# google/neural-light-transport

Hardware: AMD Instinct MI355X
Metric: rendered Mtexels/s at 1024^2 UV (full Model.call forward: U-Net + UV->camera warp); at N > 1: N collective-free replicas of this forward (weak scaling).  The data-parallel TRAIN step with the RCCL gradient all-reduce (BASELINE config 4) is `train_step`: value = Mtexels/s over all ranks, speedup_vs_o (higher is better)
Workload: dtype f32 via 3xbf16 split, 9 exact products, fp32 accumulate (the LDS-tiled encoder convs: fp32 operands as three bf16 terms on v_mfma_f32_16x16x32_bf16, every term product exact in fp32); f32 storage everywhere, every other launch native f32; 1 GPU; BASELINE config 3: dragon_specular relight+view-synth, depth0 16/depth 256, 4 frames/GPU, 1024^2 UV, k=4 obs maps, 512^2 camera warp; frames_per_gpu=4, uv=1024, k=4, cam=512, conv_algo=auto, plan=fused ends, launch=eager, two HIP streams, distinct_batches_rotated=3, launch_tape_replays=0, parallelism=dp1 (frames sharded, no forward collective), world=1, dist_world_size=1, device=cuda:0

## Files before the change

neural-light-transport_amd/csrc/conv_tile3.hip:

```cpp
#include "nlt_common.h"
#include "pack_common.h"

namespace {

typedef __attribute__((ext_vector_type(8))) __bf16 bf16x8;
typedef unsigned short u16;
typedef unsigned int u32x4 __attribute__((ext_vector_type(4)));

constexpr int TH = 8, TW = 16;
constexpr int QS2 = 272, ODD2 = 132;
constexpr int PL = 160;

template <int MODE> struct T3;
template <> struct T3<NLT_CONV_K2S1> { static constexpr int PAIRS = 2, B_UNITS = 153 * 2, B_SLOTS = 6 * PL; };
template <> struct T3<NLT_CONV_K2S2> { static constexpr int PAIRS = 1, B_UNITS = 256 * 2, B_SLOTS = 6 * QS2; };

struct Tile3P {
  const float* src; const u16* packed; const float* bias;
  float* out; float* mean_out;
  int ld, cin, frames, kobs, h, w;
  int oh, ow, cout, ldo, ldm;
  int tiles_y, tiles_x, ncc;
  int act; float alpha;
};

__device__ __forceinline__ int xcd_tile3(int b, int nblocks) {
  return (nblocks & 7) ? b : (b & 7) * (nblocks >> 3) + (b >> 3);
}

__device__ __forceinline__ unsigned cvt_pk_bf16(float a, float b) {
  typedef float f32x2_ __attribute__((ext_vector_type(2)));
  typedef __bf16 bf16x2_ __attribute__((ext_vector_type(2)));
  return __builtin_bit_cast(unsigned, __builtin_convertvector((f32x2_){a, b}, bf16x2_));
}

__device__ __forceinline__ void split2(float a, float b, unsigned& hi, unsigned& mid, unsigned& lo) {
  hi = cvt_pk_bf16(a, b);
  const float ra = a - __uint_as_float(hi << 16), rb = b - __uint_as_float(hi & 0xffff0000u);
  mid = cvt_pk_bf16(ra, rb);
  const float sa = ra - __uint_as_float(mid << 16), sb = rb - __uint_as_float(mid & 0xffff0000u);
  lo = cvt_pk_bf16(sa, sb);
}

__device__ __forceinline__ void split8(const f32x4& v0, const f32x4& v1, u32x4& hi, u32x4& mid, u32x4& lo) {
  unsigned h[4], m[4], l[4];
  split2(v0[0], v0[1], h[0], m[0], l[0]);
  split2(v0[2], v0[3], h[1], m[1], l[1]);
  split2(v1[0], v1[1], h[2], m[2], l[2]);
  split2(v1[2], v1[3], h[3], m[3], l[3]);
  hi = (u32x4){h[0], h[1], h[2], h[3]};
  mid = (u32x4){m[0], m[1], m[2], m[3]};
  lo = (u32x4){l[0], l[1], l[2], l[3]};
}


__device__ __forceinline__ int unit_half(int u) { return (u >> 3) & 1; }
__device__ __forceinline__ int unit_texel(int u) { return (u >> 4) * 8 + (u & 7); }

__device__ __forceinline__ void gather_unit(const float* sp, int ld, bool ok, long tex, int hf, f32x4& v0, f32x4& v1) {
  const float* q8 = sp + (ok ? tex : 0) * ld + 8 * hf;
  const f32x4 g0 = *reinterpret_cast<const f32x4*>(q8), g1 = *reinterpret_cast<const f32x4*>(q8 + 4);
  const f32x4 z = {0.f, 0.f, 0.f, 0.f};
  v0 = ok ? g0 : z;
  v1 = ok ? g1 : z;
}

__device__ __forceinline__ void split_store_unit(u32x4* bb, int bpl, const f32x4& v0, const f32x4& v1) {
  u32x4 hi, mid, lo;
  split8(v0, v1, hi, mid, lo);
  bb[0] = hi;
  bb[2 * bpl] = mid;
  bb[4 * bpl] = lo;
}

__device__ __forceinline__ void wave_sync() {
  __builtin_amdgcn_fence(__ATOMIC_RELEASE, "wavefront");
  __builtin_amdgcn_wave_barrier();
  __builtin_amdgcn_fence(__ATOMIC_ACQUIRE, "wavefront");
}

template <int CT>
__device__ __forceinline__ void read_a(const u32x4* A, int tile0, int lane, bf16x8 (&at)[3][CT]) {
#pragma unroll
  for (int ct = 0; ct < CT; ++ct)
#pragma unroll
    for (int t = 0; t < 3; ++t) at[t][ct] = __builtin_bit_cast(bf16x8, A[((tile0 + ct) * 3 + t) * 64 + lane]);
}

constexpr int ORDER9[9][2] = {{2, 2}, {2, 1}, {1, 2}, {2, 0}, {0, 2}, {1, 1}, {1, 0}, {0, 1}, {0, 0}};

template <int NPROD, int NR, int CT, class BFrag>
__device__ __forceinline__ void term_products(const bf16x8 (&at)[3][CT], BFrag bfrag, f32x4 (&acc)[NR][CT]) {
#pragma unroll
  for (int pi = 9 - NPROD; pi < 9; ++pi)
#pragma unroll
    for (int r = 0; r < NR; ++r)
#pragma unroll
      for (int ct = 0; ct < CT; ++ct)
        acc[r][ct] = __builtin_amdgcn_mfma_f32_16x16x32_bf16(at[ORDER9[pi][0]][ct], bfrag(ORDER9[pi][1], r), acc[r][ct], 0, 0, 0);
}

__device__ __forceinline__ f32x4 bias_act(const f32x4& acc, const f32x4& bv, int act, float alpha) {
  f32x4 v = acc + bv;
  if (act) {
#pragma unroll
    for (int c4 = 0; c4 < 4; ++c4) v[c4] = v[c4] > 0.f ? v[c4] : alpha * v[c4];
  }
  return v;
}

__host__ __device__ inline u16 bf16_rne_bits(float f) {
  union { float f; unsigned u; } x; x.f = f;
  x.u += 0x7fffu + ((x.u >> 16) & 1u);
  return (u16)(x.u >> 16);
}
__host__ __device__ inline float bf16_bits_float(u16 b) {
  union { float f; unsigned u; } x; x.u = (unsigned)b << 16;
  return x.f;
}

__global__ void pack_tile3_kernel(const float* __restrict__ wk, int cin, int cout, int tnt, long total, u16* __restrict__ wp) {
  const long idx = (long)blockIdx.x * blockDim.x + threadIdx.x;
  if (idx >= total) return;
  const int e = idx & 7, lane = (idx >> 3) & 63;
  long r = idx >> 9;
  const int term = r % 3; r /= 3;
  const int ct = r % tnt; r /= tnt;
  const int pair = r & 1; r >>= 1;
  const int ncc = cin >> 4;
  const int cc = r % ncc;
  const int g = r / ncc;
  const int kk = lane >> 4, i = lane & 15;
  const int t = pair * 2 + (kk >> 1);
  const int c = cc * 16 + (kk & 1) * 8 + e;
  const int o = (g * tnt + ct) * 16 + i;
  const float v = wk[((long)t * cin + c) * cout + o];
  const u16 hi = bf16_rne_bits(v);
  const float r1 = v - bf16_bits_float(hi);
  const u16 mid = bf16_rne_bits(r1);
  const float r2 = r1 - bf16_bits_float(mid);
  wp[idx] = term == 0 ? hi : (term == 1 ? mid : bf16_rne_bits(r2));
}

template <bool NEXT_ITEM, int NR, int CT>
__device__ __forceinline__ void epilogue(const Tile3P& p, int f, int i, int oc0, int gy0, int gx, f32x4 (&acc)[NR][CT],
                                         f32x4 (&mean)[NR][CT]) {
#pragma unroll
  for (int ct = 0; ct < CT; ++ct) {
    const int oc = oc0 + 16 * ct;
    const f32x4 bv = *reinterpret_cast<const f32x4*>(p.bias + oc);
#pragma unroll
    for (int r = 0; r < NR; ++r) {
      const int gy = gy0 + r;
      const f32x4 v = bias_act(acc[r][ct], bv, p.act, p.alpha);
      acc[r][ct] = (f32x4){0.f, 0.f, 0.f, 0.f};
      mean[r][ct] += v;
      if (gy < p.oh && gx < p.ow) {
        const long ot = ((long)(f * p.kobs + i) * p.oh + gy) * p.ow + gx;
        if (p.out) *reinterpret_cast<f32x4*>(p.out + ot * p.ldo + oc) = v;
        if (p.mean_out && i == p.kobs - 1) {
          const long mt = ((long)f * p.oh + gy) * p.ow + gx;
          *reinterpret_cast<f32x4*>(p.mean_out + mt * p.ldm + oc) = mean[r][ct] * (1.f / (float)p.kobs);
        }
      }
      if (NEXT_ITEM && i == p.kobs - 1) mean[r][ct] = (f32x4){0.f, 0.f, 0.f, 0.f};
    }
  }
}

template <int MODE>
__device__ __forceinline__ void unit_slot(int u, int& hf, int& slot, bool& st) {
  const int tx = unit_texel(u);
  hf = unit_half(u);
  if (MODE == NLT_CONV_K2S1) {
    st = tx < 153;
    slot = hf * PL + tx;
  } else {
    const int y = tx >> 5, xx = tx & 31;
    st = tx < 256;
    slot = hf * QS2 + (xx & 1) * ODD2 + y * 16 + (xx >> 1);
  }
}
template <int MODE>
__device__ __forceinline__ void unit_source(const Tile3P& p, int tx, bool st, int ty0, int tx0, bool& ok, long& tex) {
  if (MODE == NLT_CONV_K2S1) {
    const int gy = ty0 + tx / 17, gx = tx0 + tx % 17;
    ok = st && gy < p.h && gx < p.w;
    tex = (long)gy * p.w + gx;
  } else {
    const int y = tx >> 5, xx = tx & 31;
    const int gy = 2 * (ty0 + y), gx = 2 * tx0 + xx;
    ok = st && (ty0 + y) < p.oh && gx < p.w;
    tex = (long)gy * p.w + gx;
  }
}
template <int MODE, int TNT, int NPROD, int RT, int CT>
__device__ __forceinline__ void stage_products(const u32x4* A, const u32x4* B, int lane, int wm, int wn, f32x4 (&acc)[RT][CT]) {
  constexpr int BPL = MODE == NLT_CONV_K2S1 ? PL : QS2;
  const int kk = lane >> 4, j = lane & 15;
#pragma unroll
  for (int pl = 0; pl < T3<MODE>::PAIRS; ++pl) {
    bf16x8 bt[3][RT], at[3][CT];
#pragma unroll
    for (int rt = 0; rt < RT; ++rt) {
      const int y = wm * RT + rt;
      const int slot = MODE == NLT_CONV_K2S1 ? (kk & 1) * PL + (y + pl) * 17 + j + (kk >> 1)
                                             : (kk & 1) * QS2 + (kk >> 1) * ODD2 + y * 16 + j;
#pragma unroll
      for (int t = 0; t < 3; ++t) bt[t][rt] = __builtin_bit_cast(bf16x8, B[t * 2 * BPL + slot]);
    }
    read_a(A, pl * TNT + wn * CT, lane, at);
    term_products<NPROD>(at, [&](int t, int rt) { return bt[t][rt]; }, acc);
  }
}

template <int MODE, int TNT, int NPROD, int KO>
__global__ __launch_bounds__(256, 2) void conv_tile3_kernel(Tile3P p) {
  using TT = T3<MODE>;
  constexpr int WN = TNT == 4 ? 2 : 1, WM = 4 / WN, RT = TH / WM, CT = 2;
  constexpr int A_SLOTS = TT::PAIRS * TNT * 3 * 64;
  constexpr int NA = (A_SLOTS + 255) / 256, NB = (TT::B_UNITS + 255) / 256;
// ... 190 lines not shown
#pragma unroll
            for (int e = 0; e < KO; ++e)
              epilogue<true>(p, f, gi * KO + e, (g * TNT + wn * CT) * 16 + 4 * kk, ty0 + wm * RT, tx0 + j, acc[e], mean);
          }
          if (!(item_end && last_item)) store_b((q + 1) & 1);
          __syncthreads();
        }
      }
    }
    if (!last_item && ng != g) {
      copy_a(ng);
      __syncthreads();
    }
  }
}

constexpr size_t TILE3R_LDS_CU = 160 * 1024;

int tile3r_cus() {
  static const int n = [] {
    int dev = 0, v = 0;
    if (hipGetDevice(&dev) != hipSuccess) return 0;
    if (hipDeviceGetAttribute(&v, hipDeviceAttributeMultiprocessorCount, dev) != hipSuccess) return 0;
    return v;
  }();
  return n;
}

long tile3r_grid(int per_cu, int max_wg, long items) {
  long nwg = (long)tile3r_cus() * per_cu;
  if (max_wg > 0 && nwg > max_wg) nwg = max_wg;
  return nwg > items ? items : nwg;
}

int tile3r_allow_lds(const void* kernel, size_t lds, size_t (&done)[8]) {
  int dev = 0;
  if (lds <= 64 * 1024) return NLT_OK;
  if (hipGetDevice(&dev) != hipSuccess) return NLT_ERR_LAUNCH;
  if (dev >= 0 && dev < 8 && done[dev] >= lds) return NLT_OK;
  if (hipFuncSetAttribute(kernel, hipFuncAttributeMaxDynamicSharedMemorySize, (int)lds) != hipSuccess) return NLT_ERR_LAUNCH;
  if (dev >= 0 && dev < 8) done[dev] = lds;
  return NLT_OK;
}

template <int MODE, int TNT, int NPROD, int KO, int NWV>
int launch3r_k(const Tile3P& p, size_t lds, int nwg, hipStream_t s) {
  auto* k = conv_tile3r_kernel<MODE, TNT, NPROD, KO, NWV>;
  static size_t done[8] = {};
  if (tile3r_allow_lds(reinterpret_cast<const void*>(k), lds, done) != NLT_OK) return NLT_ERR_LAUNCH;
  hipLaunchKernelGGL(k, dim3((unsigned)nwg), dim3(64 * NWV), lds, s, p, p.cout / (16 * TNT));
  NLT_CHECK_LAUNCH();
  return NLT_OK;
}

template <int RT, int NPROD>
__global__ __launch_bounds__(512, 2) void conv_tile3w_kernel(Tile3P p, int ngroups, int tiles_y) {
  constexpr int TNT = 2, CT = 2, NWV = 8;
  constexpr int ROWS = RT + 1, UNITS = ROWS * 17 * 2, NB = (UNITS + 63) / 64;
  constexpr int PLW = (ROWS * 17 + 15) / 16 * 16;
  constexpr int A_SLOTS = 2 * TNT * 3 * 64;
  const int a_group = p.ncc * A_SLOTS;
  const int tid = threadIdx.x, lane = tid & 63, wave = tid >> 6;
  const int kk = lane >> 4, j = lane & 15;
  u32x4* const B = tile3r_lds + a_group + wave * (6 * PLW);
  const long in_frame = (long)p.h * p.w;
  const int tiles = p.frames * tiles_y * p.tiles_x;
  const long items = (long)tiles * ngroups;
  const int rank = xcd_tile3(blockIdx.x, gridDim.x);
  const int it0 = (int)(rank * items / gridDim.x), it1 = (int)((rank + 1) * items / gridDim.x);

  int b_lds[NB], b_hf[NB], b_tx[NB]; long b_tex[NB]; bool b_ok[NB], b_st[NB];
#pragma unroll
  for (int i = 0; i < NB; ++i) {
    b_hf[i] = unit_half(lane + 64 * i);
    b_tx[i] = unit_texel(lane + 64 * i);
    b_st[i] = b_tx[i] < ROWS * 17;
    b_lds[i] = b_hf[i] * PLW + b_tx[i];
  }
  int nf = 0, nty0 = 0, ntx0 = 0;
  auto geom = [&](int t) {
    ntx0 = (t % p.tiles_x) * TW; t /= p.tiles_x;
    nty0 = (t % tiles_y) * RT;
    nf = t / tiles_y;
#pragma unroll
    for (int i = 0; i < NB; ++i) unit_source<NLT_CONV_K2S1>(p, b_tx[i], b_st[i], nty0, ntx0, b_ok[i], b_tex[i]);
  };
  f32x4 rb[NB][2];
  auto load_b = [&](int cc, int frame) {
    const float* sp = p.src + (long)(nf * p.kobs + frame) * in_frame * p.ld + cc * 16;
#pragma unroll
    for (int n = 0; n < NB; ++n) gather_unit(sp, p.ld, b_ok[n], b_tex[n], b_hf[n], rb[n][0], rb[n][1]);
  };
  auto store_b = [&]() {
#pragma unroll
    for (int n = 0; n < NB; ++n)
      if (b_st[n]) split_store_unit(B + b_lds[n], PLW, rb[n][0], rb[n][1]);
  };

  int seg = it0;
  while (seg < it1) {
    const int g = seg / tiles;
    const int seg_end = min(it1, (g + 1) * tiles);
    {
      const u32x4* ap = reinterpret_cast<const u32x4*>(p.packed) + (long)g * a_group;
      for (int i = tid; i < a_group; i += 64 * NWV) tile3r_lds[i] = ap[i];
    }
    __syncthreads();
    int it = seg + wave;
    if (it < seg_end) {
      f32x4 acc[RT][CT], mean[RT][CT];
#pragma unroll
      for (int rt = 0; rt < RT; ++rt)
#pragma unroll
        for (int ct = 0; ct < CT; ++ct) acc[rt][ct] = mean[rt][ct] = (f32x4){0.f, 0.f, 0.f, 0.f};
      geom(it - g * tiles);
      load_b(0, 0);
      store_b();
      wave_sync();
      for (; it < seg_end; it += NWV) {
        const int f = nf, ty0 = nty0, tx0 = ntx0;
        const bool last_item = it + NWV >= seg_end;
        for (int i = 0; i < p.kobs; ++i) {
          for (int s = 0; s < p.ncc; ++s) {
            int ns = s + 1, ni = i;
            if (ns == p.ncc) { ns = 0; ++ni; }
            const bool item_end = ni == p.kobs;
            if (item_end) {
              ni = 0;
              if (!last_item) geom(it + NWV - g * tiles);
            }
            load_b(ns, ni);
            bf16x8 bt[3][ROWS];
#pragma unroll
            for (int r = 0; r < ROWS; ++r)
#pragma unroll
              for (int t = 0; t < 3; ++t)
                bt[t][r] = __builtin_bit_cast(bf16x8, B[t * 2 * PLW + (kk & 1) * PLW + r * 17 + j + (kk >> 1)]);
            wave_sync();
            const u32x4* A = tile3r_lds + s * A_SLOTS;
#pragma unroll
            for (int pl = 0; pl < 2; ++pl) {
              bf16x8 at[3][CT];
              read_a(A, pl * TNT, lane, at);
              term_products<NPROD>(at, [&](int t, int rt) { return bt[t][rt + pl]; }, acc);
            }
            if (!(item_end && last_item)) store_b();
            wave_sync();
            if (s == p.ncc - 1) epilogue<true>(p, f, i, g * TNT * 16 + 4 * kk, ty0, tx0 + j, acc, mean);
          }
        }
      }
    }
    seg = seg_end;
    if (seg < it1) __syncthreads();
  }
}

template <int RT>
int launch3w(const Tile3P& p, int nprod, int max_wg, hipStream_t s) {
  constexpr int PLW = ((RT + 1) * 17 + 15) / 16 * 16;
  const size_t lds = (size_t)p.cin * 2 * 384 + 8 * 6 * PLW * sizeof(u32x4);
  if (lds > TILE3R_LDS_CU) return NLT_ERR_UNSUPPORTED;
  const int tiles_y = (p.oh + RT - 1) / RT;
  const long nwg = tile3r_grid(1, max_wg, (long)p.frames * tiles_y * p.tiles_x * (p.cout / 32));
  if (nwg <= 0) return NLT_ERR_LAUNCH;
  auto* k = nprod == 9 ? conv_tile3w_kernel<RT, 9> : conv_tile3w_kernel<RT, 6>;
  static size_t done[2][8] = {};
  if (tile3r_allow_lds(reinterpret_cast<const void*>(k), lds, done[nprod == 9]) != NLT_OK) return NLT_ERR_LAUNCH;
  hipLaunchKernelGGL(k, dim3((unsigned)nwg), dim3(512), lds, s, p, p.cout / 32, tiles_y);
  NLT_CHECK_LAUNCH();
  return NLT_OK;
}

template <int MODE, int TNT, int KO>
int launch3r(const Tile3P& p, int nprod, int max_wg, hipStream_t s) {
  if (nprod != 6 && nprod != 9) return NLT_ERR_UNSUPPORTED;
  if (MODE == NLT_CONV_K2S1 && TNT == 2) {
    int st = launch3w<4>(p, nprod, max_wg, s);
    if (st == NLT_ERR_UNSUPPORTED) st = launch3w<2>(p, nprod, max_wg, s);
    if (st != NLT_ERR_UNSUPPORTED) return st;
  }
  const size_t lds = (size_t)p.cin * TNT * 384 + 2 * T3<MODE>::B_SLOTS * sizeof(u32x4);
  if (lds > TILE3R_LDS_CU) return NLT_ERR_UNSUPPORTED;
  const bool wide = 2 * lds > TILE3R_LDS_CU;
  const long items = (long)p.frames * p.tiles_y * p.tiles_x * (p.cout / (16 * TNT));
  const int nwg = (int)tile3r_grid(wide ? 1 : 2, max_wg, items);
  if (nwg <= 0) return NLT_ERR_LAUNCH;
  if (items >= (1l << 31)) return NLT_ERR_UNSUPPORTED;
  if (wide) return nprod == 9 ? launch3r_k<MODE, TNT, 9, KO, 8>(p, lds, nwg, s) : launch3r_k<MODE, TNT, 6, KO, 8>(p, lds, nwg, s);
  return nprod == 9 ? launch3r_k<MODE, TNT, 9, KO, 4>(p, lds, nwg, s) : launch3r_k<MODE, TNT, 6, KO, 4>(p, lds, nwg, s);
}

template <int MODE, int TNT, int KO>
int launch3k(const Tile3P& p, int nprod, hipStream_t s, int resident_wg) {
  if (resident_wg >= 0) return launch3r<MODE, TNT, KO>(p, nprod, resident_wg, s);
  const long tiles = (long)p.frames * p.tiles_y * p.tiles_x;
  const dim3 grid((unsigned)tiles, (unsigned)(p.cout / (16 * TNT)));
  if (nprod == 9) hipLaunchKernelGGL((conv_tile3_kernel<MODE, TNT, 9, KO>), grid, dim3(256), 0, s, p);
  else if (nprod == 6) hipLaunchKernelGGL((conv_tile3_kernel<MODE, TNT, 6, KO>), grid, dim3(256), 0, s, p);
  else if (KO > 1) return NLT_ERR_UNSUPPORTED;
  else if (nprod == 3) hipLaunchKernelGGL((conv_tile3_kernel<MODE, TNT, 3, 1>), grid, dim3(256), 0, s, p);
  else hipLaunchKernelGGL((conv_tile3_kernel<MODE, TNT, 1, 1>), grid, dim3(256), 0, s, p);
  NLT_CHECK_LAUNCH();
  return NLT_OK;
}

template <int MODE, int TNT>
int launch3(const Tile3P& p, int nprod, hipStream_t s, int resident_wg) {
  static const int want = [] { const char* e = getenv("NLT_TILE3_KO"); return e ? atoi(e) : 0; }();
  const int cap = want > 0 ? want : (TNT == 2 ? 4 : (MODE == NLT_CONV_K2S1 || resident_wg >= 0 ? 1 : 2));
  if (nprod >= 6) {
    if (TNT == 2 && cap >= 4 && p.kobs % 4 == 0) return launch3k<MODE, TNT, (TNT == 2 ? 4 : 1)>(p, nprod, s, resident_wg);
    if (cap >= 2 && p.kobs % 2 == 0) return launch3k<MODE, TNT, 2>(p, nprod, s, resident_wg);
  }
  return launch3k<MODE, TNT, 1>(p, nprod, s, resident_wg);
}

constexpr int S2_PITCH = 20, S2_ODD = 9, S2_PLW = 112;
constexpr int S2_A1 = 2 * 2 * 2 * 3 * 64, S2_A2 = 4 * 4 * 3 * 64;
constexpr size_t S2_LDS = (size_t)(S2_A1 + S2_A2 + 8 * 6 * S2_PLW) * sizeof(u32x4) + 96 * sizeof(float);

struct Tile3S2P {
  Tile3P a;
  const u16* packed2; const float* bias2; float* out2;
  int ldo2, act2; float alpha2;
};

template <int NPROD>
__global__ __launch_bounds__(512, 2) void conv_tile3w_s2_kernel(Tile3S2P P, int tiles_y) {
  const Tile3P& p = P.a;
  constexpr int RT = 4, CT = 2, NWV = 8, NCL = 4, NC2 = 4;
  constexpr int UNITS = 5 * 17 * 2, NB = (UNITS + 63) / 64;
  constexpr int A_SLOTS = S2_A1 / 2;
  const int tid = threadIdx.x, lane = tid & 63, wave = tid >> 6;
  const int kk = lane >> 4, j = lane & 15, yq = j >> 3, xq = j & 7;
  const u32x4* const A2 = tile3r_lds + S2_A1;
  u32x4* const B = tile3r_lds + S2_A1 + S2_A2 + wave * (6 * S2_PLW);
  float* const biasl = reinterpret_cast<float*>(tile3r_lds + S2_A1 + S2_A2 + 8 * 6 * S2_PLW);
  const long in_frame = (long)p.h * p.w;
  const int oh2 = p.h >> 1, ow2 = p.w >> 1;
  const long items = (long)p.frames * tiles_y * p.tiles_x;
  const int rank = xcd_tile3(blockIdx.x, gridDim.x);
  const int it0 = (int)(rank * items / gridDim.x), it1 = (int)((rank + 1) * items / gridDim.x);

  int b_lds[NB], b_hf[NB], b_row[NB], b_x[NB]; long b_tex[NB]; bool b_ok[NB], b_st[NB];
#pragma unroll
  for (int i = 0; i < NB; ++i) {
    const int t = unit_texel(lane + 64 * i), q = t % 17;
    b_hf[i] = unit_half(lane + 64 * i);
    b_row[i] = t / 17;
    b_x[i] = q < S2_ODD ? 2 * q : 2 * (q - S2_ODD) + 1;
    b_st[i] = t < 5 * 17;
    b_lds[i] = b_hf[i] * S2_PLW + b_row[i] * S2_PITCH + q;
  }
  int nf = 0, nty0 = 0, ntx0 = 0;
  auto geom = [&](int t) {
    ntx0 = (t % p.tiles_x) * TW; t /= p.tiles_x;
    nty0 = (t % tiles_y) * RT;
    nf = t / tiles_y;
#pragma unroll
    for (int i = 0; i < NB; ++i) {
      const int gy = nty0 + b_row[i], gx = ntx0 + b_x[i];
      b_ok[i] = b_st[i] && gy < p.h && gx < p.w;
      b_tex[i] = (long)gy * p.w + gx;
    }
  };
  f32x4 rb[NB][2];
  auto load_b = [&](int cc, int frame) {
    const float* sp = p.src + (long)(nf * p.kobs + frame) * in_frame * p.ld + cc * 16;
#pragma unroll
    for (int n = 0; n < NB; ++n) gather_unit(sp, p.ld, b_ok[n], b_tex[n], b_hf[n], rb[n][0], rb[n][1]);
  };
  auto store_b = [&]() {
#pragma unroll
    for (int n = 0; n < NB; ++n)
      if (b_st[n]) split_store_unit(B + b_lds[n], S2_PLW, rb[n][0], rb[n][1]);
  };

  {
    const u32x4* a1 = reinterpret_cast<const u32x4*>(p.packed);
    const u32x4* a2 = reinterpret_cast<const u32x4*>(P.packed2);
    for (int i = tid; i < S2_A1; i += 64 * NWV) tile3r_lds[i] = a1[i];
    for (int i = tid; i < S2_A2; i += 64 * NWV) tile3r_lds[S2_A1 + i] = a2[i];
    if (tid < 32) biasl[tid] = p.bias[tid];
    else if (tid < 96) biasl[tid] = P.bias2[tid - 32];
  }
  __syncthreads();
  int it = it0 + wave;
  if (it >= it1) return;
  const int bl0 = (kk & 1) * S2_PLW + 2 * yq * S2_PITCH + xq;
  int offx[2];
#pragma unroll
  for (int tx = 0; tx < 2; ++tx) {
    const int xx = tx + (kk >> 1);
    offx[tx] = (xx & 1) * S2_ODD + (xx >> 1);
  }
  f32x4 acc[NCL][CT], mean[NCL][CT];
#pragma unroll
  for (int c = 0; c < NCL; ++c)
#pragma unroll
    for (int ct = 0; ct < CT; ++ct) acc[c][ct] = mean[c][ct] = (f32x4){0.f, 0.f, 0.f, 0.f};
  geom(it);
  load_b(0, 0);
  store_b();
  wave_sync();
  for (; it < it1; it += NWV) {
    const int f = nf, ty0 = nty0, tx0 = ntx0;
    const bool last_item = it + NWV >= it1;
    for (int i = 0; i < p.kobs; ++i) {
      for (int s = 0; s < 2; ++s) {
        int ns = s + 1, ni = i;
        if (ns == 2) { ns = 0; ++ni; }
        const bool item_end = ni == p.kobs;
        if (item_end) {
          ni = 0;
          if (!last_item) geom(it + NWV);
        }
        load_b(ns, ni);
        bf16x8 bt[3][6];
#pragma unroll
        for (int rs = 0; rs < 3; ++rs)
#pragma unroll
          for (int tx = 0; tx < 2; ++tx)
#pragma unroll
            for (int t = 0; t < 3; ++t)
              bt[t][rs * 2 + tx] = __builtin_bit_cast(bf16x8, B[t * 2 * S2_PLW + bl0 + rs * S2_PITCH + offx[tx]]);
        wave_sync();
        const u32x4* A = tile3r_lds + s * A_SLOTS;
#pragma unroll
        for (int pl = 0; pl < 2; ++pl) {
          bf16x8 at[3][CT];
          read_a(A, pl * 2, lane, at);
          term_products<NPROD>(at, [&](int t, int c) { return bt[t][((c >> 1) + pl) * 2 + (c & 1)]; }, acc);
        }
        if (s == 1) {
          u32x4 bs[3][NCL];
#pragma unroll
          for (int c = 0; c < NCL; ++c) {
            const int gy = ty0 + 2 * yq + (c >> 1), gx = tx0 + 2 * xq + (c & 1);
            f32x4 v2[CT];
#pragma unroll
            for (int ct = 0; ct < CT; ++ct) {
              const int oc = ct * 16 + 4 * kk;
              const f32x4 v = bias_act(acc[c][ct], *reinterpret_cast<const f32x4*>(biasl + oc), p.act, p.alpha);
              acc[c][ct] = (f32x4){0.f, 0.f, 0.f, 0.f};
              mean[c][ct] += v;
              if (p.mean_out && i == p.kobs - 1 && gy < p.oh && gx < p.ow) {
                const long mt = ((long)f * p.oh + gy) * p.ow + gx;
                *reinterpret_cast<f32x4*>(p.mean_out + mt * p.ldm + oc) = mean[c][ct] * (1.f / (float)p.kobs);
              }
              if (i == p.kobs - 1) mean[c][ct] = (f32x4){0.f, 0.f, 0.f, 0.f};
              v2[ct] = v;
            }
            split8(v2[0], v2[1], bs[0][c], bs[1][c], bs[2][c]);
          }
          f32x4 acc2[NC2 / 2][1][2];
#pragma unroll
          for (int c2 = 0; c2 < NC2; ++c2) acc2[c2 >> 1][0][c2 & 1] = (f32x4){0.f, 0.f, 0.f, 0.f};
#pragma unroll
          for (int c = 0; c < NCL; ++c) {
#pragma unroll
            for (int ch = 0; ch < NC2; ch += 2) {
              bf16x8 a2[3][2];
              read_a(A2, c * NC2 + ch, lane, a2);
              term_products<NPROD>(a2, [&](int t, int) { return __builtin_bit_cast(bf16x8, bs[t][c]); }, acc2[ch >> 1]);
            }
          }
          const int oy = (ty0 >> 1) + yq, ox = (tx0 >> 1) + xq;
          if (oy < oh2 && ox < ow2) {
            const long ot = ((long)(f * p.kobs + i) * oh2 + oy) * ow2 + ox;
#pragma unroll
            for (int c2 = 0; c2 < NC2; ++c2) {
              const int oc = c2 * 16 + 4 * kk;
              *reinterpret_cast<f32x4*>(P.out2 + ot * P.ldo2 + oc) =
                  bias_act(acc2[c2 >> 1][0][c2 & 1], *reinterpret_cast<const f32x4*>(biasl + 32 + oc), P.act2, P.alpha2);
            }
          }
        }
        if (!(item_end && last_item)) store_b();
        wave_sync();
      }
    }
  }
}

int launch3w_s2(const Tile3S2P& P, int nprod, int max_wg, hipStream_t s) {
  if (S2_LDS > TILE3R_LDS_CU) return NLT_ERR_UNSUPPORTED;
  const int tiles_y = (P.a.oh + 3) / 4;
  const long items = (long)P.a.frames * tiles_y * P.a.tiles_x;
  const long nwg = tile3r_grid(1, max_wg, items);
  if (nwg <= 0) return NLT_ERR_LAUNCH;
  if (items >= (1l << 31)) return NLT_ERR_UNSUPPORTED;
  auto* k = nprod == 9 ? conv_tile3w_s2_kernel<9> : conv_tile3w_s2_kernel<6>;
  static size_t done[2][8] = {};
  if (tile3r_allow_lds(reinterpret_cast<const void*>(k), S2_LDS, done[nprod == 9]) != NLT_OK) return NLT_ERR_LAUNCH;
  hipLaunchKernelGGL(k, dim3((unsigned)nwg), dim3(512), S2_LDS, s, P, tiles_y);
  NLT_CHECK_LAUNCH();
  return NLT_OK;
}

__global__ void pack_tile3s2_kernel(const float* __restrict__ wk, int cin, int cout, long total, u16* __restrict__ wp) {
  const long idx = (long)blockIdx.x * blockDim.x + threadIdx.x;
  if (idx < total) wp[idx] = nlt_tile3s2_fragment(wk, idx, cin, cout);
}

int tile3_params(Tile3P& p, bool own_args, bool supported, bool own_layout, int ld_other, bool stride2,
                 const float* src, int ld, int cin, int frames, int kobs, int h, int w, const u16* packed, const float* bias, int cout,
                 float* out, int ldo, float* mean_out, int ldm, int act, float alpha) {
  if (!own_args || !src || !packed || !bias) return NLT_ERR_BAD_ARG;
  if (frames <= 0 || kobs <= 0 || h <= 0 || w <= 0 || cin <= 0 || cout <= 0) return NLT_ERR_BAD_ARG;
  if (!supported) return NLT_ERR_UNSUPPORTED;
  if (!own_layout || ld < cin || (ld & 3) || (out && (ldo < cout || (ldo & 3))) || (mean_out && (ldm < cout || (ldm & 3))))
    return NLT_ERR_BAD_ARG;
  if (!nlt_aligned16(src) || !nlt_aligned16(packed) || !nlt_aligned16(bias) || (out && !nlt_aligned16(out)) ||
      (mean_out && !nlt_aligned16(mean_out))) return NLT_ERR_BAD_ARG;
  if ((long long)frames * kobs * h * w * (long long)(ld > ld_other ? ld : ld_other) >= (1ll << 31)) return NLT_ERR_UNSUPPORTED;
  p.src = src; p.packed = packed; p.bias = bias; p.out = out; p.mean_out = mean_out;
  p.ld = ld; p.cin = cin; p.frames = frames; p.kobs = kobs; p.h = h; p.w = w;
  p.oh = stride2 ? h / 2 : h; p.ow = stride2 ? w / 2 : w;
  p.cout = cout; p.ldo = ldo; p.ldm = ldm; p.ncc = cin / 16; p.act = act; p.alpha = alpha;
  p.tiles_y = (p.oh + TH - 1) / TH; p.tiles_x = (p.ow + TW - 1) / TW;
  return NLT_OK;
}

}

extern "C" long nlt_conv_tile3_packed_elems(int mode, int cin, int cout, int tn) {
  if ((mode != NLT_CONV_K2S1 && mode != NLT_CONV_K2S2) || cin <= 0 || cout <= 0) return -1;
  if ((cin & 15) || (tn != 32 && tn != 64) || cout % tn) return -1;
  return (long)12 * cin * cout;
}

extern "C" int nlt_pack_conv_tile3_weights(int mode, const float* w_keras, int cin, int cout, int tn, unsigned short* packed,
                                           void* stream) {
  const long total = nlt_conv_tile3_packed_elems(mode, cin, cout, tn);
  if (total <= 0) return NLT_ERR_UNSUPPORTED;
// ... 18 lines not shown
    return tn == 64 ? launch3<NLT_CONV_K2S1, 4>(p, nprod, s, resident_wg) : launch3<NLT_CONV_K2S1, 2>(p, nprod, s, resident_wg);
  return tn == 64 ? launch3<NLT_CONV_K2S2, 4>(p, nprod, s, resident_wg) : launch3<NLT_CONV_K2S2, 2>(p, nprod, s, resident_wg);
}

extern "C" int nlt_conv_tile3_forward(int mode, int nprod, const float* src, int ld, int cin, int frames, int kobs, int h, int w,
                                      const unsigned short* packed, const float* bias, int cout, int tn,
                                      float* out, int ldo, float* mean_out, int ldm, int act, float alpha, void* stream) {
  return tile3_forward(mode, nprod, src, ld, cin, frames, kobs, h, w, packed, bias, cout, tn, out, ldo, mean_out, ldm, act, alpha,
                       -1, stream);
}

extern "C" int nlt_conv_tile3r_forward(int mode, int nprod, const float* src, int ld, int cin, int frames, int kobs, int h, int w,
                                       const unsigned short* packed, const float* bias, int cout, int tn,
                                       float* out, int ldo, float* mean_out, int ldm, int act, float alpha, int max_workgroups,
                                       void* stream) {
  if (max_workgroups < 0) return NLT_ERR_BAD_ARG;
  return tile3_forward(mode, nprod, src, ld, cin, frames, kobs, h, w, packed, bias, cout, tn, out, ldo, mean_out, ldm, act, alpha,
                       max_workgroups, stream);
}

extern "C" long nlt_conv_tile3w_s2_packed_elems(int cin2, int cout2) {
  return (cin2 == 32 && cout2 == 64) ? (long)12 * cin2 * cout2 : -1;
}

extern "C" int nlt_pack_conv_tile3w_s2_weights(const float* w_keras, int cin2, int cout2, unsigned short* packed, void* stream) {
  const long total = nlt_conv_tile3w_s2_packed_elems(cin2, cout2);
  if (total <= 0) return NLT_ERR_UNSUPPORTED;
  if (!w_keras || !packed || !nlt_aligned16(packed)) return NLT_ERR_BAD_ARG;
  hipLaunchKernelGGL(pack_tile3s2_kernel, dim3((unsigned)((total + 255) / 256)), dim3(256), 0, static_cast<hipStream_t>(stream),
                     w_keras, cin2, cout2, total, packed);
  NLT_CHECK_LAUNCH();
  return NLT_OK;
}

extern "C" long nlt_conv_tile3w_s2_lds_bytes(int cin, int cout, int cout2) {
  return (cin == 32 && cout == 32 && cout2 == 64 && S2_LDS <= TILE3R_LDS_CU) ? (long)S2_LDS : -1;
}

extern "C" int nlt_conv_tile3w_s2_forward(int nprod, const float* src, int ld, int cin, int frames, int kobs, int h, int w,
                                          const unsigned short* packed, const float* bias, int cout, float* out, int ldo,
                                          float* mean_out, int ldm, int act, float alpha,
                                          const unsigned short* packed2, const float* bias2, int cout2, float* out2, int ldo2,
                                          int act2, float alpha2, int max_workgroups, void* stream) {
  const bool own_args = packed2 && bias2 && out2 && max_workgroups >= 0 && cout2 > 0;
  const bool supported = nlt_conv_tile3w_s2_lds_bytes(cin, cout, cout2) > 0 && (nprod == 6 || nprod == 9) && !((h | w) & 1) && !out;
  const bool own_layout = ldo2 >= cout2 && !(ldo2 & 3) && nlt_aligned16(packed2) && nlt_aligned16(bias2) && nlt_aligned16(out2);
  Tile3S2P P;
  const int st = tile3_params(P.a, own_args, supported, own_layout, ldo2, false, src, ld, cin, frames, kobs, h, w, packed, bias, cout,
                              out, ldo, mean_out, ldm, act, alpha);
  if (st != NLT_OK) return st;
  P.packed2 = packed2; P.bias2 = bias2; P.out2 = out2; P.ldo2 = ldo2; P.act2 = act2; P.alpha2 = alpha2;
  return launch3w_s2(P, nprod, max_workgroups, static_cast<hipStream_t>(stream));
}
```

Measured before the change: 3692 Mtexels/s.

## Software-pipeline tile3w conv gathers across a flattened slab loop with scheduled VALU

Flattens the nested item/frame/channel-slab loops of the tile3w and tile3w_s2 conv kernels into a single slab loop driven by a SlabWalk iterator. It splits global gathers into address, issue and land phases so the next slab's loads are issued before the current slab's epilogue, and overlaps the first B-tile gather with the weight copy into LDS. It also unrolls the weight copy, hoists the bias into registers, orders B-fragment LDS reads by first use, and interleaves the split/store VALU work between MFMAs using sched_group_barrier. Optional s_memtime stamps are compiled in only under NLT_TILE3W_STAMPS. The cost is higher register pressure and unconditional stores of out-of-tile units, which now rely on static_asserts to stay inside the LDS plane.

Result: no change. 3714 Mtexels/s (median of 6 runs) (+0.6%).

```diff
diff --git a/neural-light-transport_amd/csrc/conv_tile3.hip b/neural-light-transport_amd/csrc/conv_tile3.hip
--- a/neural-light-transport_amd/csrc/conv_tile3.hip
+++ b/neural-light-transport_amd/csrc/conv_tile3.hip
@@ -65,6 +65,32 @@
   v1 = ok ? g1 : z;
 }
 
+__device__ __forceinline__ const float* gather_unit_address(const float* sp, int ld, bool ok, long tex, int hf) {
+  return sp + (ok ? tex : 0) * ld + 8 * hf;
+}
+__device__ __forceinline__ void gather_unit_issue(const float* q8, f32x4& v0, f32x4& v1) {
+  v0 = *reinterpret_cast<const f32x4*>(q8);
+  v1 = *reinterpret_cast<const f32x4*>(q8 + 4);
+}
+__device__ __forceinline__ void gather_unit_land(bool ok, f32x4& v0, f32x4& v1) {
+  const f32x4 z = {0.f, 0.f, 0.f, 0.f};
+  v0 = ok ? v0 : z;
+  v1 = ok ? v1 : z;
+}
+
+template <int NT>
+__device__ __forceinline__ void copy_weights(u32x4* dst, const u32x4* src, int n, int tid) {
+  constexpr int U = 6;
+  for (int i0 = tid; i0 < n; i0 += NT * U) {
+    u32x4 r[U];
+#pragma unroll
+    for (int u = 0; u < U; ++u) r[u] = src[min(i0 + NT * u, n - 1)];
+#pragma unroll
+    for (int u = 0; u < U; ++u)
+      if (i0 + NT * u < n) dst[i0 + NT * u] = r[u];
+  }
+}
+
 __device__ __forceinline__ void split_store_unit(u32x4* bb, int bpl, const f32x4& v0, const f32x4& v1) {
   u32x4 hi, mid, lo;
   split8(v0, v1, hi, mid, lo);
@@ -79,6 +105,60 @@
   __builtin_amdgcn_fence(__ATOMIC_ACQUIRE, "wavefront");
 }
 
+#ifdef NLT_TILE3W_STAMPS
+constexpr int T3W_NSEG = 8, T3W_NOUT = 10;
+__device__ unsigned long long* tile3w_stamp_buf = nullptr;
+__device__ __forceinline__ unsigned long long stamp_now() {
+  unsigned long long t;
+  __builtin_amdgcn_sched_barrier(0);
+  asm volatile("s_memtime %0\n\ts_waitcnt lgkmcnt(0)" : "=s"(t) : : "memory");
+  __builtin_amdgcn_sched_barrier(0);
+  return t;
+}
+struct Stamps {
+  unsigned long long t, sum[T3W_NSEG], c0, r0;
+  __device__ __forceinline__ Stamps() {
+    for (int k = 0; k < T3W_NSEG; ++k) sum[k] = 0;
+    r0 = __builtin_amdgcn_s_memrealtime();
+    c0 = t = stamp_now();
+  }
+  __device__ __forceinline__ void start() { t = stamp_now(); }
+  __device__ __forceinline__ void lap(int k) { const unsigned long long n = stamp_now(); sum[k] += n - t; t = n; }
+  __device__ __forceinline__ void write(int tid) {
+    const unsigned long long c1 = stamp_now(), r1 = __builtin_amdgcn_s_memrealtime();
+    __builtin_amdgcn_s_waitcnt(0xC07F);
+    if (tid == 0 && tile3w_stamp_buf) {
+      unsigned long long* o = tile3w_stamp_buf + (long)blockIdx.x * T3W_NOUT;
+      for (int k = 0; k < T3W_NSEG; ++k) o[k] = sum[k];
+      o[T3W_NSEG] = c1 - c0;
+      o[T3W_NSEG + 1] = r1 - r0;
+    }
+  }
+};
+#define T3W_STAMPS Stamps stamps
+#define T3W_START() stamps.start()
+#define T3W_LAP(k) stamps.lap(k)
+#define T3W_DRAIN_VM() __builtin_amdgcn_s_waitcnt(0x0F70)
+#define T3W_SLAB() (stamps.sum[T3W_NSEG - 1] += 1)
+#define T3W_WRITE(tid) stamps.write(tid)
+#else
+#define T3W_STAMPS
+#define T3W_START()
+#define T3W_LAP(k)
+#define T3W_DRAIN_VM()
+#define T3W_SLAB()
+#define T3W_WRITE(tid)
+#endif
+
+template <int NMFMA>
+__device__ __forceinline__ void spread_valu() {
+#pragma unroll
+  for (int q = 0; q < NMFMA; ++q) {
+    __builtin_amdgcn_sched_group_barrier(0x008, 1, 0);
+    __builtin_amdgcn_sched_group_barrier(0x002, 2, 0);
+  }
+}
+
 template <int CT>
 __device__ __forceinline__ void read_a(const u32x4* A, int tile0, int lane, bf16x8 (&at)[3][CT]) {
 #pragma unroll
@@ -88,6 +168,16 @@
 }
 
 constexpr int ORDER9[9][2] = {{2, 2}, {2, 1}, {1, 2}, {2, 0}, {0, 2}, {1, 1}, {1, 0}, {0, 1}, {0, 0}};
+
+constexpr int FIRST_USE_B[2][3] = {{0, 2, 1}, {2, 1, 0}};
+constexpr bool first_use_b_ok(int nprod) {
+  int n = 0;
+  bool seen[3] = {false, false, false}, ok = true;
+  for (int pi = 9 - nprod; pi < 9; ++pi)
+    if (!seen[ORDER9[pi][1]]) { seen[ORDER9[pi][1]] = true; ok = ok && FIRST_USE_B[nprod == 9][n++] == ORDER9[pi][1]; }
+  return ok && n == 3;
+}
+static_assert(first_use_b_ok(6) && first_use_b_ok(9), "FIRST_USE_B does not follow ORDER9");
 
 template <int NPROD, int NR, int CT, class BFrag>
 __device__ __forceinline__ void term_products(const bf16x8 (&at)[3][CT], BFrag bfrag, f32x4 (&acc)[NR][CT]) {
@@ -142,13 +232,13 @@
   wp[idx] = term == 0 ? hi : (term == 1 ? mid : bf16_rne_bits(r2));
 }
 
-template <bool NEXT_ITEM, int NR, int CT>
-__device__ __forceinline__ void epilogue(const Tile3P& p, int f, int i, int oc0, int gy0, int gx, f32x4 (&acc)[NR][CT],
-                                         f32x4 (&mean)[NR][CT]) {
+template <bool NEXT_ITEM, int NR, int CT, class Bias>
+__device__ __forceinline__ void epilogue_with(const Tile3P& p, Bias bias, int f, int i, int oc0, int gy0, int gx,
+                                              f32x4 (&acc)[NR][CT], f32x4 (&mean)[NR][CT]) {
 #pragma unroll
   for (int ct = 0; ct < CT; ++ct) {
     const int oc = oc0 + 16 * ct;
-    const f32x4 bv = *reinterpret_cast<const f32x4*>(p.bias + oc);
+    const f32x4 bv = bias(ct, oc);
 #pragma unroll
     for (int r = 0; r < NR; ++r) {
       const int gy = gy0 + r;
@@ -167,6 +257,11 @@
     }
   }
 }
+template <bool NEXT_ITEM, int NR, int CT>
+__device__ __forceinline__ void epilogue(const Tile3P& p, int f, int i, int oc0, int gy0, int gx, f32x4 (&acc)[NR][CT],
+                                         f32x4 (&mean)[NR][CT]) {
+  epilogue_with<NEXT_ITEM>(p, [&](int, int oc) { return *reinterpret_cast<const f32x4*>(p.bias + oc); }, f, i, oc0, gy0, gx, acc, mean);
+}
 
 template <int MODE>
 __device__ __forceinline__ void unit_slot(int u, int& hf, int& slot, bool& st) {
@@ -463,6 +558,28 @@
   NLT_CHECK_LAUNCH();
   return NLT_OK;
 }
+
+struct SlabWalk {
+  int it, i, s, f, ty, tx;
+  __device__ __forceinline__ void start(int item, int t, int tiles_x, int tiles_y) {
+    it = item; i = 0; s = 0;
+    tx = t % tiles_x; t /= tiles_x;
+    ty = t % tiles_y;
+    f = t / tiles_y;
+  }
+  __device__ __forceinline__ bool next(int ncc, int kobs, int tiles_x, int tiles_y, int end, int step) {
+    if (s + 1 < ncc) { ++s; return false; }
+    if (i + 1 < kobs) { s = 0; ++i; return false; }
+    if (it + step >= end) return false;
+    s = 0; i = 0; it += step;
+    tx += step;
+    while (tx >= tiles_x) {
+      tx -= tiles_x;
+      if (++ty == tiles_y) { ty = 0; ++f; }
+    }
+    return true;
+  }
+};
 
 template <int RT, int NPROD>
 __global__ __launch_bounds__(512, 2) void conv_tile3w_kernel(Tile3P p, int ngroups, int tiles_y) {
@@ -488,83 +605,103 @@
     b_st[i] = b_tx[i] < ROWS * 17;
     b_lds[i] = b_hf[i] * PLW + b_tx[i];
   }
-  int nf = 0, nty0 = 0, ntx0 = 0;
-  auto geom = [&](int t) {
-    ntx0 = (t % p.tiles_x) * TW; t /= p.tiles_x;
-    nty0 = (t % tiles_y) * RT;
-    nf = t / tiles_y;
-#pragma unroll
-    for (int i = 0; i < NB; ++i) unit_source<NLT_CONV_K2S1>(p, b_tx[i], b_st[i], nty0, ntx0, b_ok[i], b_tex[i]);
+  int nf = 0;
+  auto geom = [&](const SlabWalk& wk) {
+    nf = wk.f;
+#pragma unroll
+    for (int i = 0; i < NB; ++i) unit_source<NLT_CONV_K2S1>(p, b_tx[i], b_st[i], wk.ty * RT, wk.tx * TW, b_ok[i], b_tex[i]);
   };
   f32x4 rb[NB][2];
-  auto load_b = [&](int cc, int frame) {
+  const float* bq[NB];
+  auto address_b = [&](int cc, int frame) {
     const float* sp = p.src + (long)(nf * p.kobs + frame) * in_frame * p.ld + cc * 16;
 #pragma unroll
-    for (int n = 0; n < NB; ++n) gather_unit(sp, p.ld, b_ok[n], b_tex[n], b_hf[n], rb[n][0], rb[n][1]);
-  };
+    for (int n = 0; n < NB; ++n) bq[n] = gather_unit_address(sp, p.ld, b_ok[n], b_tex[n], b_hf[n]);
+  };
+  auto load_b = [&]() {
+#pragma unroll
+    for (int n = 0; n < NB; ++n) gather_unit_issue(bq[n], rb[n][0], rb[n][1]);
+  };
+  static_assert(NB * 64 / 16 * 8 <= PLW, "a copy unit past the tile must still have its slot inside the plane");
   auto store_b = [&]() {
 #pragma unroll
-    for (int n = 0; n < NB; ++n)
-      if (b_st[n]) split_store_unit(B + b_lds[n], PLW, rb[n][0], rb[n][1]);
-  };
-
+    for (int n = 0; n < NB; ++n) {
+      gather_unit_land(b_ok[n], rb[n][0], rb[n][1]);
+      split_store_unit(B + b_lds[n], PLW, rb[n][0], rb[n][1]);
+    }
+  };
+
+  T3W_STAMPS;
   int seg = it0;
   while (seg < it1) {
     const int g = seg / tiles;
     const int seg_end = min(it1, (g + 1) * tiles);
-    {
-      const u32x4* ap = reinterpret_cast<const u32x4*>(p.packed) + (long)g * a_group;
-      for (int i = tid; i < a_group; i += 64 * NWV) tile3r_lds[i] = ap[i];
-    }
+    const int it = seg + wave;
+    SlabWalk cw, lw;
+    if (it < seg_end) {
+      cw.start(it, it - g * tiles, p.tiles_x, tiles_y);
+      lw = cw;
+      geom(lw);
+      address_b(0, 0);
+      load_b();
+    }
+    copy_weights<64 * NWV>(tile3r_lds, reinterpret_cast<const u32x4*>(p.packed) + (long)g * a_group, a_group, tid);
     __syncthreads();
-    int it = seg + wave;
     if (it < seg_end) {
-      f32x4 acc[RT][CT], mean[RT][CT];
-#pragma unroll
-      for (int rt = 0; rt < RT; ++rt)
-#pragma unroll
-        for (int ct = 0; ct < CT; ++ct) acc[rt][ct] = mean[rt][ct] = (f32x4){0.f, 0.f, 0.f, 0.f};
-      geom(it - g * tiles);
-      load_b(0, 0);
+      f32x4 acc[RT][CT], mean[RT][CT], bv[CT];
+#pragma unroll
+      for (int ct = 0; ct < CT; ++ct) {
+        bv[ct] = *reinterpret_cast<const f32x4*>(p.bias + g * TNT * 16 + 4 * kk + 16 * ct);
+#pragma unroll
+        for (int rt = 0; rt < RT; ++rt) acc[rt][ct] = mean[rt][ct] = (f32x4){0.f, 0.f, 0.f, 0.f};
+      }
+      const int nslabs = (seg_end - it + NWV - 1) / NWV * p.kobs * p.ncc;
       store_b();
       wave_sync();
-      for (; it < seg_end; it += NWV) {
-        const int f = nf, ty0 = nty0, tx0 = ntx0;
-        const bool last_item = it + NWV >= seg_end;
-        for (int i = 0; i < p.kobs; ++i) {
-          for (int s = 0; s < p.ncc; ++s) {
-            int ns = s + 1, ni = i;
-            if (ns == p.ncc) { ns = 0; ++ni; }
-            const bool item_end = ni == p.kobs;
-            if (item_end) {
-              ni = 0;
-              if (!last_item) geom(it + NWV - g * tiles);
-            }
-            load_b(ns, ni);
-            bf16x8 bt[3][ROWS];
-#pragma unroll
-            for (int r = 0; r < ROWS; ++r)
-#pragma unroll
-              for (int t = 0; t < 3; ++t)
-                bt[t][r] = __builtin_bit_cast(bf16x8, B[t * 2 * PLW + (kk & 1) * PLW + r * 17 + j + (kk >> 1)]);
-            wave_sync();
-            const u32x4* A = tile3r_lds + s * A_SLOTS;
-#pragma unroll
-            for (int pl = 0; pl < 2; ++pl) {
-              bf16x8 at[3][CT];
-              read_a(A, pl * TNT, lane, at);
-              term_products<NPROD>(at, [&](int t, int rt) { return bt[t][rt + pl]; }, acc);
-            }
-            if (!(item_end && last_item)) store_b();
-            wave_sync();
-            if (s == p.ncc - 1) epilogue<true>(p, f, i, g * TNT * 16 + 4 * kk, ty0, tx0 + j, acc, mean);
+      if (lw.next(p.ncc, p.kobs, p.tiles_x, tiles_y, seg_end, NWV)) geom(lw);
+      address_b(lw.s, lw.i);
+      load_b();
+      T3W_START();
+      for (int k = 0; k < nslabs; ++k) {
+        bf16x8 bt[3][ROWS];
+#pragma unroll
+        for (int n = 0; n < 3; ++n)
+#pragma unroll
+          for (int r = 0; r < ROWS; ++r) {
+            const int t = FIRST_USE_B[NPROD == 9][n];
+            bt[t][r] = __builtin_bit_cast(bf16x8, B[t * 2 * PLW + (kk & 1) * PLW + r * 17 + j + (kk >> 1)]);
           }
-        }
+        wave_sync();
+        T3W_LAP(2);
+        const u32x4* A = tile3r_lds + cw.s * A_SLOTS;
+        bf16x8 at[2][3][CT];
+        read_a(A, 0, lane, at[0]);
+        read_a(A, TNT, lane, at[1]);
+        term_products<NPROD>(at[0], [&](int t, int rt) { return bt[t][rt]; }, acc);
+        __builtin_amdgcn_sched_barrier(0);
+        T3W_LAP(3);
+        T3W_DRAIN_VM();
+        T3W_LAP(4);
+        term_products<NPROD>(at[1], [&](int t, int rt) { return bt[t][rt + 1]; }, acc);
+        store_b();
+        spread_valu<NPROD * RT * CT>();
+        wave_sync();
+        T3W_LAP(5);
+        if (lw.next(p.ncc, p.kobs, p.tiles_x, tiles_y, seg_end, NWV)) geom(lw);
+        address_b(lw.s, lw.i);
+        load_b();
+        T3W_LAP(1);
+        if (cw.s == p.ncc - 1)
+          epilogue_with<true>(p, [&](int ct, int) { return bv[ct]; }, cw.f, cw.i, g * TNT * 16 + 4 * kk, cw.ty * RT, cw.tx * TW + j, acc, mean);
+        T3W_LAP(6);
+        cw.next(p.ncc, p.kobs, p.tiles_x, tiles_y, seg_end, NWV);
+        T3W_SLAB();
       }
     }
     seg = seg_end;
     if (seg < it1) __syncthreads();
   }
+  T3W_WRITE(tid);
 }
 
 template <int RT>
@@ -664,40 +801,52 @@
     b_st[i] = t < 5 * 17;
     b_lds[i] = b_hf[i] * S2_PLW + b_row[i] * S2_PITCH + q;
   }
-  int nf = 0, nty0 = 0, ntx0 = 0;
-  auto geom = [&](int t) {
-    ntx0 = (t % p.tiles_x) * TW; t /= p.tiles_x;
-    nty0 = (t % tiles_y) * RT;
-    nf = t / tiles_y;
+  int nf = 0;
+  auto geom = [&](const SlabWalk& wk) {
+    nf = wk.f;
 #pragma unroll
     for (int i = 0; i < NB; ++i) {
-      const int gy = nty0 + b_row[i], gx = ntx0 + b_x[i];
+      const int gy = wk.ty * RT + b_row[i], gx = wk.tx * TW + b_x[i];
       b_ok[i] = b_st[i] && gy < p.h && gx < p.w;
       b_tex[i] = (long)gy * p.w + gx;
     }
   };
   f32x4 rb[NB][2];
-  auto load_b = [&](int cc, int frame) {
+  const float* bq[NB];
+  auto address_b = [&](int cc, int frame) {
     const float* sp = p.src + (long)(nf * p.kobs + frame) * in_frame * p.ld + cc * 16;
 #pragma unroll
-    for (int n = 0; n < NB; ++n) gather_unit(sp, p.ld, b_ok[n], b_tex[n], b_hf[n], rb[n][0], rb[n][1]);
-  };
+    for (int n = 0; n < NB; ++n) bq[n] = gather_unit_address(sp, p.ld, b_ok[n], b_tex[n], b_hf[n]);
+  };
+  auto load_b = [&]() {
+#pragma unroll
+    for (int n = 0; n < NB; ++n) gather_unit_issue(bq[n], rb[n][0], rb[n][1]);
+  };
+  static_assert(NB * 64 / 16 * 8 <= 96 && 5 * S2_PITCH + 96 - 5 * 17 <= S2_PLW, "a copy unit past the tile must still have its slot inside the plane");
   auto store_b = [&]() {
 #pragma unroll
-    for (int n = 0; n < NB; ++n)
-      if (b_st[n]) split_store_unit(B + b_lds[n], S2_PLW, rb[n][0], rb[n][1]);
-  };
-
+    for (int n = 0; n < NB; ++n) {
+      gather_unit_land(b_ok[n], rb[n][0], rb[n][1]);
+      split_store_unit(B + b_lds[n], S2_PLW, rb[n][0], rb[n][1]);
+    }
+  };
+
+  const int it = it0 + wave;
+  SlabWalk cw, lw;
+  if (it < it1) {
+    cw.start(it, it, p.tiles_x, tiles_y);
+    lw = cw;
+    geom(lw);
+    address_b(0, 0);
+    load_b();
+  }
   {
-    const u32x4* a1 = reinterpret_cast<const u32x4*>(p.packed);
-    const u32x4* a2 = reinterpret_cast<const u32x4*>(P.packed2);
-    for (int i = tid; i < S2_A1; i += 64 * NWV) tile3r_lds[i] = a1[i];
-    for (int i = tid; i < S2_A2; i += 64 * NWV) tile3r_lds[S2_A1 + i] = a2[i];
+    copy_weights<64 * NWV>(tile3r_lds, reinterpret_cast<const u32x4*>(p.packed), S2_A1, tid);
+    copy_weights<64 * NWV>(tile3r_lds + S2_A1, reinterpret_cast<const u32x4*>(P.packed2), S2_A2, tid);
     if (tid < 32) biasl[tid] = p.bias[tid];
     else if (tid < 96) biasl[tid] = P.bias2[tid - 32];
   }
   __syncthreads();
-  int it = it0 + wave;
   if (it >= it1) return;
   const int bl0 = (kk & 1) * S2_PLW + 2 * yq * S2_PITCH + xq;
   int offx[2];
@@ -711,88 +860,103 @@
   for (int c = 0; c < NCL; ++c)
 #pragma unroll
     for (int ct = 0; ct < CT; ++ct) acc[c][ct] = mean[c][ct] = (f32x4){0.f, 0.f, 0.f, 0.f};
-  geom(it);
-  load_b(0, 0);
+  const int nslabs = (it1 - it + NWV - 1) / NWV * p.kobs * 2;
   store_b();
   wave_sync();
-  for (; it < it1; it += NWV) {
-    const int f = nf, ty0 = nty0, tx0 = ntx0;
-    const bool last_item = it + NWV >= it1;
-    for (int i = 0; i < p.kobs; ++i) {
-      for (int s = 0; s < 2; ++s) {
-        int ns = s + 1, ni = i;
-        if (ns == 2) { ns = 0; ++ni; }
-        const bool item_end = ni == p.kobs;
-        if (item_end) {
-          ni = 0;
-          if (!last_item) geom(it + NWV);
+  if (lw.next(2, p.kobs, p.tiles_x, tiles_y, it1, NWV)) geom(lw);
+  address_b(lw.s, lw.i);
+  load_b();
+  T3W_STAMPS;
+  for (int k = 0; k < nslabs; ++k) {
+    bf16x8 bt[3][6];
+#pragma unroll
+    for (int n = 0; n < 3; ++n)
+#pragma unroll
+      for (int rs = 0; rs < 3; ++rs)
+#pragma unroll
+        for (int tx = 0; tx < 2; ++tx) {
+          const int t = FIRST_USE_B[NPROD == 9][n];
+          bt[t][rs * 2 + tx] = __builtin_bit_cast(bf16x8, B[t * 2 * S2_PLW + bl0 + rs * S2_PITCH + offx[tx]]);
         }
-        load_b(ns, ni);
-        bf16x8 bt[3][6];
-#pragma unroll
-        for (int rs = 0; rs < 3; ++rs)
-#pragma unroll
-          for (int tx = 0; tx < 2; ++tx)
-#pragma unroll
-            for (int t = 0; t < 3; ++t)
-              bt[t][rs * 2 + tx] = __builtin_bit_cast(bf16x8, B[t * 2 * S2_PLW + bl0 + rs * S2_PITCH + offx[tx]]);
-        wave_sync();
-        const u32x4* A = tile3r_lds + s * A_SLOTS;
-#pragma unroll
-        for (int pl = 0; pl < 2; ++pl) {
-          bf16x8 at[3][CT];
-          read_a(A, pl * 2, lane, at);
-          term_products<NPROD>(at, [&](int t, int c) { return bt[t][((c >> 1) + pl) * 2 + (c & 1)]; }, acc);
+    wave_sync();
+    T3W_LAP(2);
+    const u32x4* A = tile3r_lds + cw.s * A_SLOTS;
+    bf16x8 at[2][3][CT];
+    read_a(A, 0, lane, at[0]);
+    read_a(A, 2, lane, at[1]);
+    term_products<NPROD>(at[0], [&](int t, int c) { return bt[t][(c >> 1) * 2 + (c & 1)]; }, acc);
+    __builtin_amdgcn_sched_barrier(0);
+    T3W_LAP(3);
+    T3W_DRAIN_VM();
+    T3W_LAP(4);
+    term_products<NPROD>(at[1], [&](int t, int c) { return bt[t][((c >> 1) + 1) * 2 + (c & 1)]; }, acc);
+    store_b();
+    spread_valu<NPROD * NCL * CT>();
+    wave_sync();
+    T3W_LAP(5);
+    if (lw.next(2, p.kobs, p.tiles_x, tiles_y, it1, NWV)) geom(lw);
+    address_b(lw.s, lw.i);
+    load_b();
+    T3W_LAP(1);
+    if (cw.s == 1) {
+      const int f = cw.f, i = cw.i, ty0 = cw.ty * RT, tx0 = cw.tx * TW;
+      u32x4 bs[3][NCL];
+#pragma unroll
+      for (int c = 0; c < NCL; ++c) {
+        f32x4 v2[CT];
+#pragma unroll
+        for (int ct = 0; ct < CT; ++ct) {
+          const int oc = ct * 16 + 4 * kk;
+          const f32x4 v = bias_act(acc[c][ct], *reinterpret_cast<const f32x4*>(biasl + oc), p.act, p.alpha);
+          acc[c][ct] = (f32x4){0.f, 0.f, 0.f, 0.f};
+          mean[c][ct] += v;
+          v2[ct] = v;
         }
-        if (s == 1) {
-          u32x4 bs[3][NCL];
-#pragma unroll
-          for (int c = 0; c < NCL; ++c) {
-            const int gy = ty0 + 2 * yq + (c >> 1), gx = tx0 + 2 * xq + (c & 1);
-            f32x4 v2[CT];
-#pragma unroll
-            for (int ct = 0; ct < CT; ++ct) {
-              const int oc = ct * 16 + 4 * kk;
-              const f32x4 v = bias_act(acc[c][ct], *reinterpret_cast<const f32x4*>(biasl + oc), p.act, p.alpha);
-              acc[c][ct] = (f32x4){0.f, 0.f, 0.f, 0.f};
-              mean[c][ct] += v;
-              if (p.mean_out && i == p.kobs - 1 && gy < p.oh && gx < p.ow) {
-                const long mt = ((long)f * p.oh + gy) * p.ow + gx;
-                *reinterpret_cast<f32x4*>(p.mean_out + mt * p.ldm + oc) = mean[c][ct] * (1.f / (float)p.kobs);
-              }
-              if (i == p.kobs - 1) mean[c][ct] = (f32x4){0.f, 0.f, 0.f, 0.f};
-              v2[ct] = v;
+        split8(v2[0], v2[1], bs[0][c], bs[1][c], bs[2][c]);
+      }
+      f32x4 acc2[NC2 / 2][1][2];
+#pragma unroll
+      for (int c2 = 0; c2 < NC2; ++c2) acc2[c2 >> 1][0][c2 & 1] = (f32x4){0.f, 0.f, 0.f, 0.f};
+#pragma unroll
+      for (int c = 0; c < NCL; ++c) {
+#pragma unroll
+        for (int ch = 0; ch < NC2; ch += 2) {
+          bf16x8 a2[3][2];
+          read_a(A2, c * NC2 + ch, lane, a2);
+          term_products<NPROD>(a2, [&](int t, int) { return __builtin_bit_cast(bf16x8, bs[t][c]); }, acc2[ch >> 1]);
+        }
+      }
+      const int oy = (ty0 >> 1) + yq, ox = (tx0 >> 1) + xq;
+      if (oy < oh2 && ox < ow2) {
+        const long ot = ((long)(f * p.kobs + i) * oh2 + oy) * ow2 + ox;
+#pragma unroll
+        for (int c2 = 0; c2 < NC2; ++c2) {
+          const int oc = c2 * 16 + 4 * kk;
+          *reinterpret_cast<f32x4*>(P.out2 + ot * P.ldo2 + oc) =
+              bias_act(acc2[c2 >> 1][0][c2 & 1], *reinterpret_cast<const f32x4*>(biasl + 32 + oc), P.act2, P.alpha2);
+        }
+      }
+      if (i == p.kobs - 1) {
+#pragma unroll
+        for (int c = 0; c < NCL; ++c) {
+          const int gy = ty0 + 2 * yq + (c >> 1), gx = tx0 + 2 * xq + (c & 1);
+#pragma unroll
+          for (int ct = 0; ct < CT; ++ct) {
+            const int oc = ct * 16 + 4 * kk;
+            if (p.mean_out && gy < p.oh && gx < p.ow) {
+              const long mt = ((long)f * p.oh + gy) * p.ow + gx;
+              *reinterpret_cast<f32x4*>(p.mean_out + mt * p.ldm + oc) = mean[c][ct] * (1.f / (float)p.kobs);
             }
-            split8(v2[0], v2[1], bs[0][c], bs[1][c], bs[2][c]);
-          }
-          f32x4 acc2[NC2 / 2][1][2];
-#pragma unroll
-          for (int c2 = 0; c2 < NC2; ++c2) acc2[c2 >> 1][0][c2 & 1] = (f32x4){0.f, 0.f, 0.f, 0.f};
-#pragma unroll
-          for (int c = 0; c < NCL; ++c) {
-#pragma unroll
-            for (int ch = 0; ch < NC2; ch += 2) {
-              bf16x8 a2[3][2];
-              read_a(A2, c * NC2 + ch, lane, a2);
-              term_products<NPROD>(a2, [&](int t, int) { return __builtin_bit_cast(bf16x8, bs[t][c]); }, acc2[ch >> 1]);
-            }
-          }
-          const int oy = (ty0 >> 1) + yq, ox = (tx0 >> 1) + xq;
-          if (oy < oh2 && ox < ow2) {
-            const long ot = ((long)(f * p.kobs + i) * oh2 + oy) * ow2 + ox;
-#pragma unroll
-            for (int c2 = 0; c2 < NC2; ++c2) {
-              const int oc = c2 * 16 + 4 * kk;
-              *reinterpret_cast<f32x4*>(P.out2 + ot * P.ldo2 + oc) =
-                  bias_act(acc2[c2 >> 1][0][c2 & 1], *reinterpret_cast<const f32x4*>(biasl + 32 + oc), P.act2, P.alpha2);
-            }
+            mean[c][ct] = (f32x4){0.f, 0.f, 0.f, 0.f};
           }
         }
-        if (!(item_end && last_item)) store_b();
-        wave_sync();
       }
     }
-  }
+    T3W_LAP(6);
+    cw.next(2, p.kobs, p.tiles_x, tiles_y, it1, NWV);
+    T3W_SLAB();
+  }
+  T3W_WRITE(tid);
 }
 
 int launch3w_s2(const Tile3S2P& P, int nprod, int max_wg, hipStream_t s) {
@@ -917,3 +1081,9 @@
   P.packed2 = packed2; P.bias2 = bias2; P.out2 = out2; P.ldo2 = ldo2; P.act2 = act2; P.alpha2 = alpha2;
   return launch3w_s2(P, nprod, max_workgroups, static_cast<hipStream_t>(stream));
 }
+
+#ifdef NLT_TILE3W_STAMPS
+extern "C" int nlt_tile3w_stamp_buffer(void* buf) {
+  return hipMemcpyToSymbol(HIP_SYMBOL(tile3w_stamp_buf), &buf, sizeof(buf)) == hipSuccess ? NLT_OK : NLT_ERR_LAUNCH;
+}
+#endif
```
